# Richard-coder/uvio

Hardware: AMD Instinct MI355X
Metric: VIO frames/sec (track+propagate+update) at clones x feats (higher is better)
Workload: dtype f64

## Files before the change

include/uvio_hp.h:

```cpp
#ifndef UVIO_HP_H
#define UVIO_HP_H

#include <stddef.h>
#include <stdint.h>

#ifdef __cplusplus
extern "C" {
#endif

#define UVIO_HP_OK 0
#define UVIO_HP_E_ARG (-1)
#define UVIO_HP_E_STATE (-2)
#define UVIO_HP_E_DEVICE (-3)
#define UVIO_HP_E_NUMERIC (-4)
#define UVIO_HP_E_CONFIG (-5)
#define UVIO_HP_E_ORDER (-6)
#define UVIO_HP_E_CAPACITY (-7)
#define UVIO_HP_E_INTERNAL (-8)

#define UVIO_HP_MAX_CAMS 4
#define UVIO_HP_MAX_ANCHORS 16


typedef struct {
// ... 156 lines not shown
int uvio_hp_marginalize_slam(uvio_hp_t *h);
int uvio_hp_marginalize_old_clone(uvio_hp_t *h);
int uvio_hp_uwb_update_single(uvio_hp_t *h, double t, uint64_t anchor_id, double range, int *applied);

typedef int (*uvio_hp_allreduce_fn)(double *buf, size_t count, void *user);
int uvio_hp_shard_unique_id(uint8_t id[128]);
int uvio_hp_shard_init_rccl(uvio_hp_t *h, int rank, int world, const uint8_t id[128], int min_features);
int uvio_hp_shard_init_host(uvio_hp_t *h, int rank, int world, uvio_hp_allreduce_fn fn, void *user,
                            int min_features);
int uvio_hp_shard_partition(const int *rows, int n, int world, int *bounds);

int uvio_hp_debug_last_msckf(uvio_hp_t *h, uint64_t *ids, double *pG, int *status, double *chi2, int cap, int *n);
int uvio_hp_debug_frame_feats(uvio_hp_t *h, int *kind, uint64_t *ids, double *pG, int *status, double *chi2, int cap,
                              int *n);
int uvio_hp_ekf_update(double *P, int N, const int *H_index, int n, const double *H, int r,
                       const double *res, double sigma2, double *dx_out);
int uvio_hp_msckf_compressed_update(double *P, int N, const int *H_index, int n, const double *H, int m,
                                    const double *res, double sigma2, double *dx_out);
int uvio_hp_compress(const double *A, int m, int n, double *R_out);
int uvio_hp_undistort(int model, const double cam[8], int n, const float *uv, float *uvn, uint8_t *ambiguous);
int uvio_hp_debug_grid_order(const uint8_t *resp, const int *off, int ncell, int kmax, int depth, int *arrangement,
                             int *top);
int uvio_hp_debug_clahe(const uint8_t *img, int w, int h, int stride, uint8_t *out);
int uvio_hp_debug_grid_stats(uvio_hp_t *h, uint64_t *cells, uint64_t *introsort_cells);

#ifdef __cplusplus
}
#endif
#endif
```

uvio_amd/_native.py:

```python
import ctypes as C
import os

ROOT = os.path.dirname(os.path.dirname(os.path.abspath(__file__)))
LIB_PATH = os.environ.get("UVIO_HP_LIB", os.path.join(ROOT, "uvio_amd", "libuvio_hp.so"))

MAX_CAMS = 4
MAX_ANCHORS = 16

OK = 0
E_ARG, E_STATE, E_DEVICE, E_NUMERIC, E_CONFIG, E_ORDER, E_CAPACITY, E_INTERNAL = -1, -2, -3, -4, -5, -6, -7, -8
ERRNAMES = {0: "OK", -1: "E_ARG", -2: "E_STATE", -3: "E_DEVICE", -4: "E_NUMERIC", -5: "E_CONFIG", -6: "E_ORDER",
            -7: "E_CAPACITY", -8: "E_INTERNAL"}


class Camera(C.Structure):
    _fields_ = [("model", C.c_int), ("width", C.c_int), ("height", C.c_int), ("intrinsics", C.c_double * 8),
                ("q_ItoC", C.c_double * 4), ("p_IinC", C.c_double * 3)]


class Anchor(C.Structure):
    _fields_ = [("id", C.c_uint64), ("fix", C.c_int), ("p_AinG", C.c_double * 3), ("const_bias", C.c_double),
                ("dist_bias", C.c_double), ("cov_diag", C.c_double * 5)]


# ... 99 lines not shown
    ("get_tracks", _I, [C.c_void_p, _I, _P(C.c_uint64), _P(C.c_float), _I, _P(_I)]),
    ("get_pyramid", _I, [C.c_void_p, _I, _I, _P(_I), _P(_I), _P(C.c_uint8), _P(C.c_int16), C.c_size_t]),
    ("debug_last_msckf", _I, [C.c_void_p, _P(C.c_uint64), _P(_D), _P(_I), _P(_D), _I, _P(_I)]),
    ("debug_frame_feats", _I, [C.c_void_p, _P(_I), _P(C.c_uint64), _P(_D), _P(_I), _P(_D), _I, _P(_I)]),
    ("ekf_update", _I, [_P(_D), _I, _P(_I), _I, _P(_D), _I, _P(_D), _D, _P(_D)]),
    ("msckf_compressed_update", _I, [_P(_D), _I, _P(_I), _I, _P(_D), _I, _P(_D), _D, _P(_D)]),
    ("compress", _I, [_P(_D), _I, _I, _P(_D)]),
    ("undistort", _I, [_I, _P(_D), _I, _P(C.c_float), _P(C.c_float), _P(C.c_uint8)]),
    ("set_state", _I, [C.c_void_p, _P(_D), _P(_D), _I, _P(_D), _I, _I]),
    ("propagate_and_clone", _I, [C.c_void_p, _D]),
    ("msckf_update", _I, [C.c_void_p, _I, _P(C.c_uint64), _P(_I), _P(FeatMeas), _P(FeatResult)]),
    ("slam_update", _I, [C.c_void_p, _I, _P(C.c_uint64), _P(_I), _P(FeatMeas), _P(FeatResult)]),
    ("slam_delayed_init", _I, [C.c_void_p, _I, _P(C.c_uint64), _P(_I), _P(FeatMeas), _P(FeatResult)]),
    ("slam_change_anchors", _I, [C.c_void_p]),
    ("marginalize_slam", _I, [C.c_void_p]),
    ("marginalize_old_clone", _I, [C.c_void_p]),
    ("uwb_update_single", _I, [C.c_void_p, _D, C.c_uint64, _D, _P(_I)]),
    ("shard_unique_id", _I, [_P(C.c_uint8)]),
    ("shard_init_rccl", _I, [C.c_void_p, _I, _I, _P(C.c_uint8), _I]),
    ("shard_init_host", _I, [C.c_void_p, _I, _I, C.c_void_p, C.c_void_p, _I]),
    ("shard_partition", _I, [_P(_I), _I, _I, _P(_I)]),
    ("debug_grid_order", _I, [_P(C.c_uint8), _P(_I), _I, _I, _I, _P(_I), _P(_I)]),
    ("debug_clahe", _I, [_P(C.c_uint8), _I, _I, _I, _P(C.c_uint8)]),
    ("debug_grid_stats", _I, [C.c_void_p, _P(C.c_uint64), _P(C.c_uint64)]),
]

ALLREDUCE_FN = C.CFUNCTYPE(C.c_int, _P(_D), C.c_size_t, C.c_void_p)

EXPORTED = ["uvio_hp_" + s[0] for s in SIGNATURES]


MISSING = set()


def bind(lib, prefix, names=None):
    ab_old = os.environ.get("UVIO_HP_AB_OLD") == "1" and "UVIO_HP_LIB" in os.environ
    for name, res, args in SIGNATURES:
        if names is not None and name not in names:
            continue
        if ab_old and prefix == "uvio_hp_" and not hasattr(lib, prefix + name):
            MISSING.add(name)
            continue
        f = getattr(lib, prefix + name)
        f.restype = res
        f.argtypes = args
    if MISSING:
# ... 32 lines not shown
```

uvio_amd/csrc/capi.cpp:

```cpp
#include <cstring>
#include <string>

#include "engine.h"

using namespace uvhp;

struct uvio_hp {
  Engine *e = nullptr;
  std::string err;
  std::string fatal;
};

static std::string internal_error(const uvio_hp *h, const std::exception &ex) {
  std::string m = std::string("internal error: ") + ex.what();
  if (h && h->e && h->e->stage()[0]) m += std::string(" (in ") + h->e->stage() + ")";
  return m;
}

#define HP_GUARD(h, body)                                    \
  try {                                                      \
    if ((h) && (h)->e) HP_HIP(hipSetDevice((h)->e->device())); \
    body                                                     \
  } catch (const HpError &ex) {                              \
    if (h) (h)->err = ex.what();                             \
// ... 344 lines not shown
}

int uvio_hp_undistort(int model, const double cam[8], int n, const float *uv, float *uvn, uint8_t *ambiguous) {
  try {
    return Engine::undistort_standalone(model, cam, n, uv, uvn, ambiguous);
  } catch (const HpError &ex) {
    return ex.code;
  } catch (...) {
    return UVIO_HP_E_DEVICE;
  }
}

int uvio_hp_debug_grid_order(const uint8_t *resp, const int *off, int ncell, int kmax, int depth, int *arrangement,
                             int *top) {
  try {
    return Engine::grid_order_standalone(resp, off, ncell, kmax, depth, arrangement, top);
  } catch (const HpError &ex) {
    return ex.code;
  } catch (...) {
    return UVIO_HP_E_DEVICE;
  }
}

int uvio_hp_debug_clahe(const uint8_t *img, int w, int h, int stride, uint8_t *out) {
  try {
    return Engine::clahe_standalone(img, w, h, stride, out);
  } catch (const HpError &ex) {
    return ex.code;
  } catch (...) {
    return UVIO_HP_E_DEVICE;
  }
}

int uvio_hp_debug_grid_stats(uvio_hp_t *h, uint64_t *cells, uint64_t *introsort_cells) {
  if (!h) return UVIO_HP_E_ARG;
  unsigned long long c = 0;
  unsigned long long i = 0;
  HP_GUARD(h, if (h->e->tracker()) h->e->tracker()->grid_stats(&c, &i);)
  if (cells) *cells = c;
  if (introsort_cells) *introsort_cells = i;
  return 0;
}

}
```

uvio_amd/csrc/engine.h:

```cpp
#pragma once
#include <chrono>
#include <atomic>
#include <functional>
#include <map>
#include <memory>
#include <mutex>
#include <stdexcept>
#include <unordered_map>
#include <algorithm>
#include <cstdlib>
#include <vector>

#include "hp_common.h"
#include "hprof.h"
#include "kernels.h"
#include "pool.h"
#include "tracker.h"

namespace uvhp {

enum VKind { V_IMU = 0, V_VEC = 1, V_QUAT = 2, V_POSE = 3, V_LANDMARK = 4, V_ANCHOR = 5 };

struct Var {
  VKind kind;
// ... 335 lines not shown
  const Var &imu() const { return *imu_; }
  int cov_dim() const { return N_; }
  void get_cov(double *out, int ld);
  int state_vector(double *out, int cap, int *meta, int meta_cap, int *nvars, bool fej = false);
  uvio_hp_timing_t timing() const { return timing_; }
  std::vector<double> clone_times() const;

  void set_kernel_timing(int period) {
    ktime_period_ = period;
    kprof_.on = period > 0 && frames_ % period == 0;
  }
  void kernel_stats(bool flush, uvio_hp_kstat_t *out, int cap, int *n);

  void shard_init_rccl(int rank, int world, const uint8_t id[128], int min_features);
  void shard_init_host(int rank, int world, uvio_hp_allreduce_fn fn, void *user, int min_features);

  static int ekf_update_standalone(double *P, int N, const int *H_index, int n, const double *H, int r, const double *res,
                                   double sigma2, double *dx_out, bool compress = false);
  static int compress_standalone(const double *A, int m, int n, double *R_out);
  static int undistort_standalone(int model, const double cam[8], int n, const float *uv, float *uvn, uint8_t *amb);
  static int grid_order_standalone(const uint8_t *resp, const int *off, int ncell, int kmax, int depth,
                                   int *arrangement, int *top);
  static int clahe_standalone(const uint8_t *img, int w, int h, int stride, uint8_t *out);

 private:
  uvio_hp_options_t o_;
  int device_;
  DeviceBufs d_;
  double timestamp_ = -1;
  VarP imu_, calib_dt_, dw_, da_, tg_, qg_, qa_, p_IinU_;
  std::map<double, VarP> clones_;
  std::unordered_map<size_t, VarP> slam_;
  std::unordered_map<size_t, VarP> calib_pose_, calib_intr_;
  std::unordered_map<size_t, VarP> anchors_;
  CamParams cams_[UVIO_HP_MAX_CAMS];
  std::vector<VarP> vars_;
  int N_ = 0;
  long long p_epoch_ = 0;
  double early_prop_s_ = 0.0;
  std::mutex imu_mtx_;
  std::vector<ImuSample> imu_data_;
  bool have_last_prop_time_offset_ = false;
  double last_prop_time_offset_ = 0;
  std::unique_ptr<Tracker> tracker_;
  NodeSlabs db_nodes_;
  DbMap db_{SlabAlloc<std::pair<const size_t, FeatP>>(&db_nodes_)};
// ... 240 lines not shown
```

uvio_amd/csrc/engine_state.cpp:

```cpp
#include <sys/stat.h>

#include <algorithm>
#include <cstdio>
#include <cstring>

#include "engine.h"

namespace uvhp {

void Var::update(const double *dx) {
  if (kind == V_IMU || kind == V_POSE || kind == V_QUAT) {
    quat_boxplus(val, dx);
    for (int i = 3; i < size; i++) val[i + 1] += dx[i];
  } else {
    for (int i = 0; i < size; i++) val[i] += dx[i];
  }
}

void Var::xyz(bool getfej, double *o) const {
  const double *p = getfej ? fej : val;
  switch (rep) {
    case 0:
    case 2:
      o[0] = p[0]; o[1] = p[1]; o[2] = p[2];
// ... 950 lines not shown
  const size_t n = (size_t)w * h;
  ProbeScope ps;
  uint8_t *d_src = ps.alloc<uint8_t>(n), *d_img = ps.alloc<uint8_t>(n);
  int16_t *d_der = ps.alloc<int16_t>(2 * n);
  PyrJob job{};
  job.ncam = 1;
  job.method = 2;
  job.p[0].levels = 1;
  job.p[0].w[0] = w;
  job.p[0].h[0] = h;
  job.p[0].img[0] = d_img;
  job.p[0].der[0] = d_der;
  job.src[0] = d_src;
  job.stride[0] = w;
  job.clahe[0] = ps.alloc<uint8_t>(kClaheLutBytes);
  HP_HIP(hipMemcpy2DAsync(d_src, w, img, stride, w, h, hipMemcpyHostToDevice, ps.s));
  launch_pyramids(ps.s, job);
  HP_HIP(hipGetLastError());
  HP_HIP(hipMemcpyAsync(out, d_img, n, hipMemcpyDeviceToHost, ps.s));
  HP_HIP(hipStreamSynchronize(ps.s));
  return 0;
}

}
```

uvio_amd/csrc/kernels.h:

```cpp
#pragma once
#include <hip/hip_runtime.h>

#include <cstdint>

#include "hp_math.h"
#include "kprof.h"

namespace uvhp {

constexpr int kMaxMeasPerFeat = 64;
constexpr int kMaxVarsPerFeat = 48;
constexpr int kMaxCams = 4;

struct DClone {
  double R[9], p[3];
  double Rf[9], pf[3];
  int pid;
  int canon;
  int pad[2];
};

struct DCam {
  double R_ItoC[9], p_IinC[3];
  CamParams cam;
// ... 54 lines not shown
  const double *xv;
  int *gate_out;
};

void launch_cov_propagate(hipStream_t s, double *P, int ld, int N, int s0, int p, const int *iold, int q,
                          const double *Phi, const double *Q, double *T, const int *rows = nullptr);
void launch_clone(hipStream_t s, double *P, int ld, int N, int src0, int dt_id, const double *dnc_dev, int do_dt);
bool launch_prop_clone(hipStream_t s, double *P, int ld, int N, int s0, int p, const int *iold, int q,
                       const double *Phi, const double *Q, double *T, int src0, int dt_id, const double *dnc_dev,
                       int do_dt);
void launch_marginalize(hipStream_t s, const double *P, double *Pout, int ld, int N, int m0, int ms);
void launch_compact(hipStream_t s, const double *P, double *Pout, int ld, int Nn, const int *src);
void launch_marginalize_multi(hipStream_t s, const double *P, double *Pout, int ld, int Nn, const int *src);
void launch_check_diag(hipStream_t s, const double *P, int ld, int N, int *neg);

void launch_feature_linearize(hipStream_t s, const DBatchParams &bp, const DFeat *feats, const DMeas *meas,
                              const DVar *vars, const DClone *clones, const DCam *cams, const double *P,
                              const double *chi2_table, double *H_all, DFeatOut *out, int max_meas, int max_nf);
void launch_chi2_batch(hipStream_t s, const DBatchParams &bp, const DFeat *feats, const double *P, const int *hidx,
                       double *H_all, int m, double *T_all, const double *chi2_table, DFeatOut *out, int max_rows_f,
                       int *acc_count, double *pcan = nullptr,
                       double **sbuf = nullptr, size_t *sbuf_cap = nullptr);
size_t feature_lds_bytes(int max_meas, int max_nf);

void launch_gram(hipStream_t s, const double *A, int m, int ncol, int ldh, double *partials, int *nchunks_out);
int gram_num_chunks(int m);
void launch_shard_pack(hipStream_t s, const double *partials, int nch, int ncol, const DFeatOut *fout, int nf,
                       const int *acc, double *buf);
void launch_shard_unpack(hipStream_t s, const double *buf, int ncol, int *acc);
void launch_gram_reduce_chol(hipStream_t s, const double *partials, int nchunks, int ncol, double *R, int ldr);

constexpr int kMaxEkfRows = 255;
constexpr int kMaxDynLds = 152 * 1024;
constexpr int kUwbMaxRanges = 16;
struct DUwbState {
  double q[4], p[3];
  double pU[3];
  double anc[kUwbMaxRanges][5];
  double range[kUwbMaxRanges];
  int id_imu, id_cal;
  int id_anc[kUwbMaxRanges];
  int nr;
};
void launch_uwb_row(hipStream_t s, DUwbState *st, int j, const double *prev, double *h, double *region);
void launch_uwb_M(hipStream_t s, const double *P, int ldp, int N, const double *h, const int *hidx, int n, double *M);
void launch_uwb_update(hipStream_t s, double *P, int ldp, int N, const double *M, const double *h, const int *hidx,
// ... 175 lines not shown
```

uvio_amd/csrc/kernels_feat.hip:

```cpp
#include <stdexcept>
#include <string>

#include "kernels.h"

namespace uvhp {

__device__ __forceinline__ double wave_sum(double v) {
#pragma unroll
  for (int o = 32; o > 0; o >>= 1) v += __shfl_xor(v, o, 64);
  return v;
}
__device__ __forceinline__ void wave_sync() {
  __builtin_amdgcn_fence(__ATOMIC_RELEASE, "wavefront");
  __builtin_amdgcn_wave_barrier();
  __builtin_amdgcn_fence(__ATOMIC_ACQUIRE, "wavefront");
}
template <int NV>
__device__ __forceinline__ void ordered_sum(double *red, const double *v, int lane, int m, double *out) {
  wave_sync();
#pragma unroll
  for (int k = 0; k < NV; k++) red[lane * NV + k] = v[k];
  wave_sync();
  if (lane < NV) {
    double s = 0.0;
// ... 92 lines not shown
#pragma unroll
      for (int i = k + 1; i < 3; i++) s += A[3 * i + j] * A[3 * i + j];
      cn[j] = s;
    }
  }
  double y[3] = {0, 0, 0};
#pragma unroll
  for (int i = 2; i >= 0; i--) {
    if (i < rank) {
      double v = b[i];
#pragma unroll
      for (int k = i + 1; k < 3; k++)
        if (k < rank) v -= A[3 * i + k] * y[k];
      y[i] = v / A[3 * i + i];
    }
  }
#pragma unroll
  for (int i = 0; i < 3; i++)
#pragma unroll
    for (int j = 0; j < 3; j++)
      if (perm[i] == j) x[j] = y[i];
}

__device__ void singular_values3(const double *A, double *sv) {
  double a[3][3];
  for (int i = 0; i < 3; i++)
    for (int j = 0; j < 3; j++) a[i][j] = A[i] * A[j] + A[3 + i] * A[3 + j] + A[6 + i] * A[6 + j];
  for (int sweep = 0; sweep < 60; sweep++) {
    double off = a[0][1] * a[0][1] + a[0][2] * a[0][2] + a[1][2] * a[1][2];
    if (off < 1e-300 || off <= 1e-36 * (a[0][0] * a[0][0] + a[1][1] * a[1][1] + a[2][2] * a[2][2])) break;
    for (int p = 0; p < 2; p++)
      for (int q = p + 1; q < 3; q++) {
        if (a[p][q] == 0) continue;
        double theta = (a[q][q] - a[p][p]) / (2 * a[p][q]);
        double t = (theta >= 0 ? 1.0 : -1.0) / (fabs(theta) + sqrt(theta * theta + 1));
        double c = 1 / sqrt(t * t + 1), s = t * c;
        for (int k = 0; k < 3; k++) {
          double akp = a[k][p], akq = a[k][q];
          a[k][p] = c * akp - s * akq;
          a[k][q] = s * akp + c * akq;
        }
        for (int k = 0; k < 3; k++) {
          double apk = a[p][k], aqk = a[q][k];
          a[p][k] = c * apk - s * aqk;
          a[q][k] = s * apk + c * aqk;
        }
      }
// ... 80 lines not shown
        w1[q] = a1[q];
        w2[q] = a2[q];
        w3[q] = a3[q];
      } else {
        w1[q] = __shfl(a1[q / TPC], base + q % TPC, 64);
        w2[q] = __shfl(a2[q / TPC], base + q % TPC, 64);
        w3[q] = __shfl(a3[q / TPC], base + q % TPC, 64);
      }
    }
    const double s1 = (w1[0] + w1[1]) + (w1[2] + w1[3]);
    const double s2 = (w2[0] + w2[1]) + (w2[2] + w2[3]);
    const double s3 = (w3[0] + w3[1]) + (w3[2] + w3[3]);
    const double u1 = b1 * s1;
    const double u2 = b2 * (s2 - g21 * u1);
    const double u3 = b3 * (s3 - g31 * u1 - g32 * u2);
#pragma unroll 4
    for (int k = part; k < rows; k += TPC) {
      double *p = Hl + (size_t)k * ldl + j;
      *p -= V[k * 3] * u1 + V[k * 3 + 1] * u2 + V[k * 3 + 2] * u3;
    }
  }
}

struct FeatShared {
  double p_FinA[3], p_FinG[3], p_FinA_fej[3], p_FinG_fej[3];
  int status;
  int nrows_out;
  double beta[3];
  double chi2;
};

__host__ __device__ inline size_t feat_lds_doubles(int max_meas, int max_nf) {
  int rows = 2 * max_meas;
  size_t n = 0;
  n += (size_t)rows * (max_nf + 1);
  n += (size_t)rows * 3;
  n += (size_t)rows * 3;
  n += (size_t)max_nf;
  n += 64;
  return n;
}
size_t feature_lds_bytes(int max_meas, int max_nf) { return feat_lds_doubles(max_meas, max_nf) * sizeof(double); }

__global__ void __launch_bounds__(256) k_feature(DBatchParams bp, const DFeat *__restrict__ feats,
                                                 const DMeas *__restrict__ meas, const DVar *__restrict__ vars,
                                                 const DClone *__restrict__ clones, const DCam *__restrict__ cams,
                                                 const double *__restrict__ P, const double *__restrict__ chi2_table,
                                                 double *__restrict__ H_all, DFeatOut *__restrict__ out, int max_meas,
                                                 int max_nf) {
  extern __shared__ double lds[];
  __shared__ FeatShared sh;
  long long *tsp = bp.dbg_ts ? bp.dbg_ts + (size_t)blockIdx.x * 16 : nullptr;
#define FEAT_TS(k) \
  if (tsp && threadIdx.x == 0) tsp[k] = clock64();
  __shared__ int canon2loc[512];
  __shared__ double red[9 * 64 + 16];
  const int f = blockIdx.x;
  const DFeat F = feats[f];
  const int m = F.nmeas, rows = 2 * m, nf = F.nf, ldl = nf + 1;
  const int tid = threadIdx.x, lane = tid & 63, wave = tid >> 6;
  const DMeas *Ms = meas + F.meas_off;

  double *Hl = lds;
  double *Hf = Hl + (size_t)2 * max_meas * (max_nf + 1);
  double *V = Hf + 2 * max_meas * 3;
  int *loc2pid = (int *)(V + 2 * max_meas * 3);

  FEAT_TS(0)
  for (int j = tid; j <= bp.n_canon; j += 256) canon2loc[j] = -1;
  for (int e = tid; e < rows * ldl; e += 256) Hl[e] = 0.0;
  __syncthreads();
  for (int e = tid; e < F.nvar * 8; e += 256) {
    const DVar dv = vars[F.var_off + (e >> 3)];
    const int k = e & 7;
    if (k < dv.size) {
      loc2pid[dv.loc + k] = dv.pid + k;
      if (dv.canon >= 0) canon2loc[dv.canon + k] = dv.loc + k;
    }
  }
  if (tid == 0) {
    sh.status = 0;
    double pin[3], pinf[3];
    for (int k = 0; k < 3; k++) pin[k] = F.p_in[k], pinf[k] = F.p_in_fej[k];
    if (F.mode == 3 && bp.tri_in) {
      const DFeatOut &t = bp.tri_in[f];
      for (int k = 0; k < 3; k++) pin[k] = t.p_FinA[k], pinf[k] = t.p_FinG[k];
      if (t.status == 1 || t.status == 2) sh.status = 1;
    }
    if (F.mode == 1 && bp.xv && F.lm_pid >= 0) {
      const double *v = bp.xv + F.lm_pid;
      if (F.rep == 4) {
        pin[0] = (1 / v[2]) * v[0];
        pin[1] = (1 / v[2]) * v[1];
        pin[2] = 1 / v[2];
        for (int k = 0; k < 3; k++) pinf[k] = pin[k];
      } else {
        for (int k = 0; k < 3; k++) pin[k] = v[k];
      }
    }
    for (int k = 0; k < 3; k++) {
// ... 364 lines not shown
        if (bp.calib_ext)
          for (int j = 0; j < 6; j++)
            row[F.lc_anchor_ext + j] +=
                dz_dpfg[3 * i] * Hcal[j] + dz_dpfg[3 * i + 1] * Hcal[6 + j] + dz_dpfg[3 * i + 2] * Hcal[12 + j];
      }
      if (bp.calib_ext && mm.lc_ext >= 0) {
        double pc[3] = {p_FinCi[0] - ck.p_IinC[0], p_FinCi[1] - ck.p_IinC[1], p_FinCi[2] - ck.p_IinC[2]}, Sc[9];
        skew(pc, Sc);
        for (int j = 0; j < 3; j++) {
          row[mm.lc_ext + j] += dz_dpfc[3 * i] * Sc[j] + dz_dpfc[3 * i + 1] * Sc[3 + j] + dz_dpfc[3 * i + 2] * Sc[6 + j];
          row[mm.lc_ext + 3 + j] += dz_dpfc[3 * i + j];
        }
      }
      if (bp.calib_intr && mm.lc_intr >= 0)
        for (int j = 0; j < 8; j++) row[mm.lc_intr + j] = dzeta[8 * i + j];
      row[nf] = (i == 0) ? res0 : res1;
      if (F.mode == 1)
        for (int j = 0; j < ncolf; j++) row[F.lm_loc + j] = hf[j];
    }
  }
  __syncthreads();

  FEAT_TS(3)
  int r0 = 0;
  if (status0 == 0 && F.mode != 1) {
    if (wave == 0) {
      for (int c = 0; c < 3; c++) {
        double ss = 0.0;
        for (int i = c + lane; i < rows; i += 64) {
          double x = Hf[i * 3 + c];
          ss += x * x;
        }
        ss = wave_sum(ss);
        const double x0 = Hf[c * 3 + c];
        const double alpha = (x0 > 0) ? -sqrt(ss) : sqrt(ss);
        for (int i = lane; i < rows; i += 64) {
          V[i * 3 + c] = (i < c) ? 0.0 : (i == c) ? (x0 - alpha) : Hf[i * 3 + c];
          if (i >= c) Hf[i * 3 + c] = (i == c) ? alpha : 0.0;
        }
        const double vn = ss - x0 * x0 + (x0 - alpha) * (x0 - alpha);
        const double b = (vn > 0) ? 2.0 / vn : 0.0;
        if (lane == 0) sh.beta[c] = b;
        wave_sync();
        for (int j = c + 1; j < 3; j++) {
          double d = 0.0;
          for (int i = c + lane; i < rows; i += 64) d += V[i * 3 + c] * Hf[i * 3 + j];
          d = b * wave_sum(d);
          for (int i = c + lane; i < rows; i += 64) Hf[i * 3 + j] -= d * V[i * 3 + c];
        }
        wave_sync();
      }
      double g0 = 0.0, g1 = 0.0, g2 = 0.0;
      for (int i = lane; i < rows; i += 64) {
        const double a = V[i * 3], bq = V[i * 3 + 1], cq = V[i * 3 + 2];
        g0 += bq * a;
        g1 += cq * a;
        g2 += cq * bq;
      }
      g0 = wave_sum(g0);
      g1 = wave_sum(g1);
      g2 = wave_sum(g2);
      if (lane == 0) red[0] = g0, red[1] = g1, red[2] = g2;
      if (F.mode == 3) FEAT_TS(8)
    }
    __syncthreads();
    if (F.mode == 3) FEAT_TS(9)
    const double b1 = sh.beta[0], b2 = sh.beta[1], b3 = sh.beta[2];
    const double g21 = red[0], g31 = red[1], g32 = red[2];
    if (ldl <= 64)
      ns_apply<4>(Hl, V, rows, ldl, tid, b1, b2, b3, g21, g31, g32);
    else if (ldl <= 128)
      ns_apply<2>(Hl, V, rows, ldl, tid, b1, b2, b3, g21, g31, g32);
    else
      ns_apply<1>(Hl, V, rows, ldl, tid, b1, b2, b3, g21, g31, g32);
    if (F.mode == 3) FEAT_TS(10)
    __syncthreads();
    r0 = 3;
  }
  const int R = rows - r0;

  FEAT_TS(4)
  FEAT_TS(5)
  const int status = sh.status;
  FEAT_TS(6)
  const int out_r0 = (F.mode == 0) ? 3 : 0;
  const int nrows_out = max(rows - out_r0, 0);
  {
    const int nc = bp.n_canon + 1;
    int lcs[8];
#pragma unroll
    for (int q = 0; q < 8; q++) {
      const int j = lane + 64 * q;
      lcs[q] = (status != 0 || j >= nc) ? -1 : (j == bp.n_canon) ? nf : canon2loc[j];
    }
    for (int i = wave; i < nrows_out; i += 4) {
      const double *src = Hl + (size_t)(out_r0 + i) * ldl;
      double *dst = H_all + (size_t)(F.row_off + i) * bp.ldh;
#pragma unroll
      for (int q = 0; q < 8; q++) {
        const int j = lane + 64 * q;
        if (j < nc) dst[j] = (lcs[q] >= 0) ? src[lcs[q]] : 0.0;
      }
    }
  }
  if (tid == 0) {
    DFeatOut o;
    for (int k = 0; k < 3; k++) {
      o.p_FinA[k] = sh.p_FinA[k];
      o.p_FinG[k] = sh.p_FinG[k];
    }
    o.chi2 = -1.0;
    for (int k = 0; k < 9; k++) o.HfR[k] = (F.mode >= 2 && status0 == 0) ? Hf[(k / 3) * 3 + (k % 3)] : 0.0;
    o.status = status;
    o.rows = status == 0 ? nrows_out : 0;
    out[f] = o;
    if (bp.gate_out) *bp.gate_out = (status == 0) ? 1 : 0;
  }
  FEAT_TS(7)
#undef FEAT_TS
}

void launch_feature_linearize(hipStream_t s, const DBatchParams &bp, const DFeat *feats, const DMeas *meas,
                              const DVar *vars, const DClone *clones, const DCam *cams, const double *P,
                              const double *chi2_table, double *H_all, DFeatOut *out, int max_meas, int max_nf) {
  if (bp.nfeat <= 0) return;
  if (bp.n_canon >= 512 || max_meas > 64)
    throw std::runtime_error("k_feature: n_canon " + std::to_string(bp.n_canon) + " / measurements per feature " +
                             std::to_string(max_meas) + " beyond the kernel's limits (511 / 64)");
  size_t bytes = feature_lds_bytes(max_meas, max_nf);
  static int granted = -1;
  if (granted < 0) granted = set_dyn_lds((const void *)k_feature, 156 * 1024);
  if (bytes > 64 * 1024 && (int)bytes > granted)
    throw std::runtime_error("k_feature needs " + std::to_string(bytes) + " B of LDS, granted " + std::to_string(granted));
  hipLaunchKernelGGL(k_feature, dim3(bp.nfeat), dim3(256), bytes, s, bp, feats, meas, vars, clones, cams, P,
                     chi2_table, H_all, out, max_meas, max_nf);
}

__device__ __forceinline__ unsigned retri_hash(unsigned long long k, int cap) {
  k ^= k >> 33;
  k *= 0xff51afd7ed558ccdull;
  k ^= k >> 33;
  return (unsigned)(k & (unsigned long long)(cap - 1));
}
__device__ int retri_find(const unsigned long long *keys, int cap, unsigned long long id) {
  unsigned h = retri_hash(id, cap);
  for (int p = 0; p < cap; p++, h = (h + 1) & (cap - 1)) {
    const unsigned long long k = keys[h];
    if (k == id) return (int)h;
    if (k == kRetriEmpty) return -1;
  }
  return -1;
}
__device__ int retri_insert(unsigned long long *keys, int cap, unsigned long long id) {
  unsigned h = retri_hash(id, cap);
  for (int p = 0; p < cap; p++, h = (h + 1) & (cap - 1)) {
    const unsigned long long prev = atomicCAS(&keys[h], kRetriEmpty, id);
    if (prev == kRetriEmpty || prev == id) return (int)h;
  }
// ... 143 lines not shown
```

uvio_amd/manager.py:

```python
import ctypes as C

import numpy as np

from . import _native as N


def load_options(yaml_path=None, **overrides):
    lib = N.load()
    opts = N.Options()
    N.check(lib.uvio_hp_options_default(C.byref(opts)), what="options_default")
    if yaml_path is not None:
        N.check(lib.uvio_hp_options_load(yaml_path.encode(), C.byref(opts)), what="options_load(%s)" % yaml_path)
    apply_overrides(opts, overrides)
    return opts


def _mask_ptrs(masks, ncam):
    mk = [None if m is None else np.ascontiguousarray(m, dtype=np.uint8) for m in masks]
    ptrs = [C.POINTER(C.c_uint8)() if m is None else m.ctypes.data_as(C.POINTER(C.c_uint8)) for m in mk]
    return mk, (C.POINTER(C.c_uint8) * ncam)(*ptrs)


def apply_overrides(opts, overrides):
    for k, v in overrides.items():
# ... 393 lines not shown
    N.check(lib.uvio_hp_compress(_dp(A), m, nc - 1, _dp(R)), what="uvio_hp_compress")
    return R


def grid_order(cells, kmax=0, depth=-1):
    lib = N.load()
    off = np.zeros(len(cells) + 1, dtype=np.int32)
    for i, c in enumerate(cells):
        off[i + 1] = off[i] + len(c)
    resp = np.zeros(max(int(off[-1]), 1), dtype=np.uint8)
    for i, c in enumerate(cells):
        resp[off[i]:off[i + 1]] = np.asarray(c, dtype=np.int64)
    arr = np.zeros(max(int(off[-1]), 1), dtype=np.int32)
    top = np.full(max(len(cells) * kmax, 1), -1, dtype=np.int32)
    ip = C.POINTER(C.c_int)
    rc = lib.uvio_hp_debug_grid_order(resp.ctypes.data_as(C.POINTER(C.c_uint8)), off.ctypes.data_as(ip), len(cells),
                                      kmax, depth, arr.ctypes.data_as(ip), top.ctypes.data_as(ip))
    N.check(rc, what="uvio_hp_debug_grid_order")
    arrs = [arr[off[i]:off[i + 1]].copy() for i in range(len(cells))]
    tops = [top[i * kmax:i * kmax + min(kmax, len(c))].copy() for i, c in enumerate(cells)] if kmax > 0 else None
    return arrs, tops


def clahe(img):
    lib = N.load()
    img = np.asarray(img)
    if img.ndim != 2 or img.dtype != np.uint8:
        raise ValueError("clahe: a 2-D uint8 image")
    if img.strides[1] != 1 or img.strides[0] < img.shape[1]:
        img = np.ascontiguousarray(img)
    h, w = img.shape
    out = np.zeros((h, w), dtype=np.uint8)
    bp = C.POINTER(C.c_uint8)
    rc = lib.uvio_hp_debug_clahe(img.ctypes.data_as(bp), w, h, img.strides[0], out.ctypes.data_as(bp))
    N.check(rc, what="uvio_hp_debug_clahe")
    return out


def undistort(cam, uv, return_ambiguous=False):
    lib = N.load()
    uv = np.ascontiguousarray(uv, dtype=np.float32).reshape(-1, 2)
    out = np.zeros_like(uv)
    amb = np.zeros(uv.shape[0], dtype=np.uint8)
    intr = np.array(cam.intrinsics[:], dtype=np.float64)
    fp = C.POINTER(C.c_float)
    rc = lib.uvio_hp_undistort(int(cam.model), _dp(intr), uv.shape[0], uv.ctypes.data_as(fp), out.ctypes.data_as(fp),
# ... 4 lines not shown
```

Baseline: 1067.

## Apply nullspace projection from registers and scatter directly to H_all

Adds a register-resident path for the three-reflector Householder nullspace projection in k_feature. Each wave holds a quarter of the rows for up to four 64-column blocks and exchanges partial reflector sums through LDS, then writes projected rows straight into canonical H_all columns instead of writing back to LDS and running a separate scatter pass. k_feature is templated on row and column capacity and dispatched from a table, with an env var to force the old LDS path. A standalone probe API is added for testing, and the register footprint per template may affect occupancy.

```diff
diff --git a/include/uvio_hp.h b/include/uvio_hp.h
--- a/include/uvio_hp.h
+++ b/include/uvio_hp.h
@@ -202,6 +202,9 @@
 int uvio_hp_debug_grid_order(const uint8_t *resp, const int *off, int ncell, int kmax, int depth, int *arrangement,
                              int *top);
 int uvio_hp_debug_clahe(const uint8_t *img, int w, int h, int stride, uint8_t *out);
+int uvio_hp_debug_ns_project(const double *A, int rows, int ldl, const double *V, const double beta[3],
+                             const double g[3], const int *loc2canon, int n_canon, int out_r0, int variant,
+                             int status, double *out);
 int uvio_hp_debug_grid_stats(uvio_hp_t *h, uint64_t *cells, uint64_t *introsort_cells);
 
 #ifdef __cplusplus
diff --git a/uvio_amd/_native.py b/uvio_amd/_native.py
--- a/uvio_amd/_native.py
+++ b/uvio_amd/_native.py
@@ -145,6 +145,7 @@
     ("shard_partition", _I, [_P(_I), _I, _I, _P(_I)]),
     ("debug_grid_order", _I, [_P(C.c_uint8), _P(_I), _I, _I, _I, _P(_I), _P(_I)]),
     ("debug_clahe", _I, [_P(C.c_uint8), _I, _I, _I, _P(C.c_uint8)]),
+    ("debug_ns_project", _I, [_P(_D), _I, _I, _P(_D), _P(_D), _P(_D), _P(_I), _I, _I, _I, _I, _P(_D)]),
     ("debug_grid_stats", _I, [C.c_void_p, _P(C.c_uint64), _P(C.c_uint64)]),
 ]
 
diff --git a/uvio_amd/csrc/capi.cpp b/uvio_amd/csrc/capi.cpp
--- a/uvio_amd/csrc/capi.cpp
+++ b/uvio_amd/csrc/capi.cpp
@@ -390,6 +390,18 @@
   }
 }
 
+int uvio_hp_debug_ns_project(const double *A, int rows, int ldl, const double *V, const double beta[3],
+                             const double g[3], const int *loc2canon, int n_canon, int out_r0, int variant,
+                             int status, double *out) {
+  try {
+    return Engine::ns_project_standalone(A, rows, ldl, V, beta, g, loc2canon, n_canon, out_r0, variant, status, out);
+  } catch (const HpError &ex) {
+    return ex.code;
+  } catch (...) {
+    return UVIO_HP_E_DEVICE;
+  }
+}
+
 int uvio_hp_debug_clahe(const uint8_t *img, int w, int h, int stride, uint8_t *out) {
   try {
     return Engine::clahe_standalone(img, w, h, stride, out);
diff --git a/uvio_amd/csrc/engine.h b/uvio_amd/csrc/engine.h
--- a/uvio_amd/csrc/engine.h
+++ b/uvio_amd/csrc/engine.h
@@ -381,6 +381,9 @@
   static int grid_order_standalone(const uint8_t *resp, const int *off, int ncell, int kmax, int depth,
                                    int *arrangement, int *top);
   static int clahe_standalone(const uint8_t *img, int w, int h, int stride, uint8_t *out);
+  static int ns_project_standalone(const double *A, int rows, int ldl, const double *V, const double beta[3],
+                                   const double g[3], const int *loc2canon, int n_canon, int out_r0, int variant,
+                                   int status, double *out);
 
  private:
   uvio_hp_options_t o_;
diff --git a/uvio_amd/csrc/engine_state.cpp b/uvio_amd/csrc/engine_state.cpp
--- a/uvio_amd/csrc/engine_state.cpp
+++ b/uvio_amd/csrc/engine_state.cpp
@@ -996,4 +996,38 @@
   return 0;
 }
 
-}
+int Engine::ns_project_standalone(const double *A, int rows, int ldl, const double *V, const double beta[3],
+                                  const double g[3], const int *loc2canon, int n_canon, int out_r0, int variant,
+                                  int status, double *out) {
+  if (!A || !V || !beta || !g || !loc2canon || !out || variant < 0 || variant > 4 || out_r0 < 0 || n_canon < 0)
+    return UVIO_HP_E_ARG;
+  if (rows < 2 || rows > 128 || (rows & 1) || ldl < 2 || ldl > 512 || n_canon >= 512) return UVIO_HP_E_CAPACITY;
+  if (variant >= 2 && (ldl > 64 * variant || rows < 12)) return UVIO_HP_E_ARG;
+  std::vector<char> seen(n_canon, 0);
+  for (int j = 0; j + 1 < ldl; j++) {
+    const int c = loc2canon[j];
+    if (c >= n_canon || (c >= 0 && seen[c]++)) return UVIO_HP_E_ARG;
+  }
+  if (loc2canon[ldl - 1] != n_canon) return UVIO_HP_E_ARG;
+  int ndev = 0;
+  if (hipGetDeviceCount(&ndev) != hipSuccess || ndev < 1) return UVIO_HP_E_DEVICE;
+  const size_t nA = (size_t)rows * ldl, nout = (size_t)std::max(rows - out_r0, 0) * (n_canon + 1);
+  if (nout == 0) return 0;
+  ProbeScope ps;
+  double *d_A = ps.alloc<double>(nA), *d_work = ps.alloc<double>(nA), *d_V = ps.alloc<double>((size_t)rows * 3);
+  double *d_bg = ps.alloc<double>(6), *d_out = ps.alloc<double>(nout);
+  int *d_map = ps.alloc<int>(ldl);
+  const double bg[6] = {beta[0], beta[1], beta[2], g[0], g[1], g[2]};
+  HP_HIP(hipMemcpyAsync(d_A, A, sizeof(double) * nA, hipMemcpyHostToDevice, ps.s));
+  HP_HIP(hipMemcpyAsync(d_V, V, sizeof(double) * rows * 3, hipMemcpyHostToDevice, ps.s));
+  HP_HIP(hipMemcpyAsync(d_bg, bg, sizeof(bg), hipMemcpyHostToDevice, ps.s));
+  HP_HIP(hipMemcpyAsync(d_map, loc2canon, sizeof(int) * ldl, hipMemcpyHostToDevice, ps.s));
+  HP_HIP(hipMemsetAsync(d_out, 0xff, sizeof(double) * nout, ps.s));
+  launch_ns_project_probe(ps.s, d_A, d_work, d_V, d_bg, d_map, rows, ldl, n_canon, out_r0, variant, status, d_out);
+  HP_HIP(hipGetLastError());
+  HP_HIP(hipMemcpyAsync(out, d_out, sizeof(double) * nout, hipMemcpyDeviceToHost, ps.s));
+  HP_HIP(hipStreamSynchronize(ps.s));
+  return 0;
+}
+
+}
diff --git a/uvio_amd/csrc/kernels.h b/uvio_amd/csrc/kernels.h
--- a/uvio_amd/csrc/kernels.h
+++ b/uvio_amd/csrc/kernels.h
@@ -100,6 +100,9 @@
                        int *acc_count, double *pcan = nullptr,
                        double **sbuf = nullptr, size_t *sbuf_cap = nullptr);
 size_t feature_lds_bytes(int max_meas, int max_nf);
+void launch_ns_project_probe(hipStream_t s, const double *d_A, double *d_work, const double *d_V, const double *d_bg,
+                             const int *d_loc2canon, int rows, int ldl, int n_canon, int out_r0, int variant,
+                             int status, double *d_out);
 
 void launch_gram(hipStream_t s, const double *A, int m, int ncol, int ldh, double *partials, int *nchunks_out);
 int gram_num_chunks(int m);
diff --git a/uvio_amd/csrc/kernels_feat.hip b/uvio_amd/csrc/kernels_feat.hip
--- a/uvio_amd/csrc/kernels_feat.hip
+++ b/uvio_amd/csrc/kernels_feat.hip
@@ -138,7 +138,7 @@
       if (perm[i] == j) x[j] = y[i];
 }
 
-__device__ void singular_values3(const double *A, double *sv) {
+__device__ __forceinline__ void singular_values3(const double *A, double *sv) {
   double a[3][3];
   for (int i = 0; i < 3; i++)
     for (int j = 0; j < 3; j++) a[i][j] = A[i] * A[j] + A[3 + i] * A[3 + j] + A[6 + i] * A[6 + j];
@@ -265,6 +265,237 @@
   }
 }
 
+
+__host__ __device__ inline int ns_reg_cb(int rows, int ldl, int cbmax) {
+  return (rows < 12 || ldl <= 64 || ldl > 64 * cbmax) ? 0 : (ldl + 63) / 64;
+}
+
+__device__ __forceinline__ void ns_zero_cols(const int *canon2loc, int n_canon, double *dst0, int ldh, int nrows_out,
+                                             int w, int nw, int lane) {
+  bool z[8];
+#pragma unroll
+  for (int q = 0; q < 8; q++) {
+    const int j = lane + 64 * q;
+    z[q] = j < n_canon && canon2loc[j] < 0;
+  }
+  for (int i = w; i < nrows_out; i += nw) {
+    double *dst = dst0 + (size_t)i * ldh;
+#pragma unroll
+    for (int q = 0; q < 8; q++)
+      if (z[q]) dst[lane + 64 * q] = 0.0;
+  }
+}
+
+template <int RQ, int CB>
+__device__ __forceinline__ void ns_reg_load(double (&a)[RQ][CB], const double *Hl, int nq, int ldl, int part, int col0) {
+  auto row = [&](int k) {
+    const double *src = Hl + (size_t)(4 * k + part) * ldl;
+#pragma unroll
+    for (int c = 0; c < CB; c++) a[k][c] = src[min(col0 + 64 * c, ldl - 1)];
+  };
+#pragma unroll
+  for (int k0 = 0; k0 < RQ; k0 += 4) {
+    if (k0 + 4 <= nq) {
+#pragma unroll
+      for (int k = k0; k < k0 + 4; k++) row(k);
+    } else {
+#pragma unroll
+      for (int k = k0; k < k0 + 4; k++) {
+        if (k < nq) {
+          row(k);
+        } else {
+#pragma unroll
+          for (int c = 0; c < CB; c++) a[k][c] = 0.0;
+        }
+      }
+    }
+  }
+}
+
+template <int RQ, int CB>
+__device__ __forceinline__ void ns_reg_apply(double (&a)[RQ][CB], double *Hl, const double *V, int rows, int ldl,
+                                             int part, int col0, double b1, double b2, double b3, double g21,
+                                             double g31, double g32, const int (&cn)[CB], double *dst0, int ldh,
+                                             int out_r0, long long *ts) {
+  const int rows4 = rows & ~3, nq = rows4 >> 2;
+  double a1[CB], a2[CB], a3[CB];
+#pragma unroll
+  for (int c = 0; c < CB; c++) a1[c] = a2[c] = a3[c] = 0.0;
+  auto sum_row = [&](int k) {
+    const double *v = V + (4 * k + part) * 3;
+    const double v1 = v[0], v2 = v[1], v3 = v[2];
+#pragma unroll
+    for (int c = 0; c < CB; c++) {
+      a1[c] += v1 * a[k][c];
+      a2[c] += v2 * a[k][c];
+      a3[c] += v3 * a[k][c];
+    }
+  };
+#pragma unroll
+  for (int k0 = 0; k0 < RQ; k0 += 4) {
+    if (k0 + 4 <= nq) {
+#pragma unroll
+      for (int k = k0; k < k0 + 4; k++) sum_row(k);
+    } else {
+#pragma unroll
+      for (int k = k0; k < k0 + 4; k++)
+        if (k < nq) sum_row(k);
+    }
+  }
+  if (part == 0)
+    for (int r = rows4; r < rows; r++) {
+      const double v1 = V[r * 3], v2 = V[r * 3 + 1], v3 = V[r * 3 + 2];
+#pragma unroll
+      for (int c = 0; c < CB; c++) {
+        const int j = col0 + 64 * c;
+        const double x = (j < ldl) ? Hl[(size_t)r * ldl + j] : 0.0;
+        a1[c] += v1 * x;
+        a2[c] += v2 * x;
+        a3[c] += v3 * x;
+      }
+    }
+  double *xch = Hl;
+#pragma unroll
+  for (int c = 0; c < CB; c++) {
+    const int j = col0 + 64 * c;
+    if (j < ldl) {
+      xch[(size_t)(3 * part) * ldl + j] = a1[c];
+      xch[(size_t)(3 * part + 1) * ldl + j] = a2[c];
+      xch[(size_t)(3 * part + 2) * ldl + j] = a3[c];
+    }
+  }
+  __syncthreads();
+  if (ts && threadIdx.x == 0) ts[11] = clock64();
+  double u1[CB], u2[CB], u3[CB];
+#pragma unroll
+  for (int c = 0; c < CB; c++) {
+    const double *w = xch + min(col0 + 64 * c, ldl - 1);
+    const double s1 = (w[0] + w[(size_t)3 * ldl]) + (w[(size_t)6 * ldl] + w[(size_t)9 * ldl]);
+    const double s2 = (w[(size_t)ldl] + w[(size_t)4 * ldl]) + (w[(size_t)7 * ldl] + w[(size_t)10 * ldl]);
+    const double s3 = (w[(size_t)2 * ldl] + w[(size_t)5 * ldl]) + (w[(size_t)8 * ldl] + w[(size_t)11 * ldl]);
+    u1[c] = b1 * s1;
+    u2[c] = b2 * (s2 - g21 * u1[c]);
+    u3[c] = b3 * (s3 - g31 * u1[c] - g32 * u2[c]);
+  }
+  asm volatile("" ::: "memory");
+  auto out_row = [&](int k) {
+    const int r = 4 * k + part;
+    const double v1 = V[r * 3], v2 = V[r * 3 + 1], v3 = V[r * 3 + 2];
+    double *dst = dst0 + ((ptrdiff_t)r - out_r0) * ldh;
+#pragma unroll
+    for (int c = 0; c < CB; c++) {
+      const double x = a[k][c] - (v1 * u1[c] + v2 * u2[c] + v3 * u3[c]);
+      if (r >= out_r0 && cn[c] >= 0) dst[cn[c]] = x;
+    }
+  };
+#pragma unroll
+  for (int k0 = 0; k0 < RQ; k0 += 4) {
+    if (k0 + 4 <= nq) {
+#pragma unroll
+      for (int k = k0; k < k0 + 4; k++) out_row(k);
+    } else {
+#pragma unroll
+      for (int k = k0; k < k0 + 4; k++)
+        if (k < nq) out_row(k);
+    }
+  }
+  const int rt = rows4 + part - 2;
+  if (part >= 2 && rt < rows && rt >= out_r0) {
+    const double v1 = V[rt * 3], v2 = V[rt * 3 + 1], v3 = V[rt * 3 + 2];
+    double *dst = dst0 + (size_t)(rt - out_r0) * ldh;
+#pragma unroll
+    for (int c = 0; c < CB; c++)
+      if (cn[c] >= 0) dst[cn[c]] = Hl[(size_t)rt * ldl + col0 + 64 * c] - (v1 * u1[c] + v2 * u2[c] + v3 * u3[c]);
+  }
+}
+
+__device__ __forceinline__ void ns_reflectors(double *Hf, double *V, int rows, int lane, double *beta, double *g) {
+  for (int c = 0; c < 3; c++) {
+    double ss = 0.0;
+    for (int i = c + lane; i < rows; i += 64) {
+      double x = Hf[i * 3 + c];
+      ss += x * x;
+    }
+    ss = wave_sum(ss);
+    const double x0 = Hf[c * 3 + c];
+    const double alpha = (x0 > 0) ? -sqrt(ss) : sqrt(ss);
+    for (int i = lane; i < rows; i += 64) {
+      V[i * 3 + c] = (i < c) ? 0.0 : (i == c) ? (x0 - alpha) : Hf[i * 3 + c];
+      if (i >= c) Hf[i * 3 + c] = (i == c) ? alpha : 0.0;
+    }
+    const double vn = ss - x0 * x0 + (x0 - alpha) * (x0 - alpha);
+    const double b = (vn > 0) ? 2.0 / vn : 0.0;
+    if (lane == 0) beta[c] = b;
+    wave_sync();
+    for (int j = c + 1; j < 3; j++) {
+      double d = 0.0;
+      for (int i = c + lane; i < rows; i += 64) d += V[i * 3 + c] * Hf[i * 3 + j];
+      d = b * wave_sum(d);
+      for (int i = c + lane; i < rows; i += 64) Hf[i * 3 + j] -= d * V[i * 3 + c];
+    }
+    wave_sync();
+  }
+  double g0 = 0.0, g1 = 0.0, g2 = 0.0;
+  for (int i = lane; i < rows; i += 64) {
+    const double a = V[i * 3], bq = V[i * 3 + 1], cq = V[i * 3 + 2];
+    g0 += bq * a;
+    g1 += cq * a;
+    g2 += cq * bq;
+  }
+  g0 = wave_sum(g0);
+  g1 = wave_sum(g1);
+  g2 = wave_sum(g2);
+  if (lane == 0) g[0] = g0, g[1] = g1, g[2] = g2;
+}
+
+template <int RQ, int CB>
+__device__ __forceinline__ void ns_project_reg(double *Hl, double *Hf, double *V, double *beta, double *g,
+                                               int rows, int ldl, int tid, const int *canon2loc,
+                                               const int *loc2canon, int n_canon, double *dst0, int ldh, int out_r0,
+                                               long long *ts) {
+  const int lane = tid & 63, wave = tid >> 6, part = wave, col0 = lane, nf = ldl - 1;
+  const int nq = (rows & ~3) >> 2;
+  double a[RQ][CB];
+  int cn[CB];
+#pragma unroll
+  for (int c = 0; c < CB; c++) {
+    const int j = col0 + 64 * c;
+    cn[c] = (j < nf) ? loc2canon[j] : (j == nf) ? n_canon : -1;
+  }
+  if (wave == 0 && Hf) {
+    ns_reflectors(Hf, V, rows, lane, beta, g);
+    if (ts && lane == 0) ts[8] = clock64();
+  }
+  ns_reg_load<RQ, CB>(a, Hl, nq, ldl, part, col0);
+  if (wave != 0) ns_zero_cols(canon2loc, n_canon, dst0, ldh, max(rows - out_r0, 0), wave - 1, 3, lane);
+  __syncthreads();
+  if (ts && tid == 0) ts[9] = clock64();
+  ns_reg_apply<RQ, CB>(a, Hl, V, rows, ldl, part, col0, beta[0], beta[1], beta[2], g[0], g[1], g[2], cn, dst0, ldh,
+                       out_r0, ts);
+  if (ts && tid == 0) ts[10] = clock64();
+}
+
+__device__ __forceinline__ void ns_write_rows_lds(const double *Hl, int ldl, const int *canon2loc, int n_canon,
+                                                  int status, double *dst0, int ldh, int out_r0, int nrows_out,
+                                                  int lane, int wave) {
+  const int nc = n_canon + 1, nf = ldl - 1;
+  int lcs[8];
+#pragma unroll
+  for (int q = 0; q < 8; q++) {
+    const int j = lane + 64 * q;
+    lcs[q] = (status != 0 || j >= nc) ? -1 : (j == n_canon) ? nf : canon2loc[j];
+  }
+  for (int i = wave; i < nrows_out; i += 4) {
+    const double *src = Hl + (size_t)(out_r0 + i) * ldl;
+    double *dst = dst0 + (size_t)i * ldh;
+#pragma unroll
+    for (int q = 0; q < 8; q++) {
+      const int j = lane + 64 * q;
+      if (j < nc) dst[j] = (lcs[q] >= 0) ? src[lcs[q]] : 0.0;
+    }
+  }
+}
+
 struct FeatShared {
   double p_FinA[3], p_FinG[3], p_FinA_fej[3], p_FinG_fej[3];
   int status;
@@ -285,12 +516,13 @@
 }
 size_t feature_lds_bytes(int max_meas, int max_nf) { return feat_lds_doubles(max_meas, max_nf) * sizeof(double); }
 
+template <int RQ, int CBMAX>
 __global__ void __launch_bounds__(256) k_feature(DBatchParams bp, const DFeat *__restrict__ feats,
                                                  const DMeas *__restrict__ meas, const DVar *__restrict__ vars,
                                                  const DClone *__restrict__ clones, const DCam *__restrict__ cams,
                                                  const double *__restrict__ P, const double *__restrict__ chi2_table,
                                                  double *__restrict__ H_all, DFeatOut *__restrict__ out, int max_meas,
-                                                 int max_nf) {
+                                                 int max_nf, int ns_lds) {
   extern __shared__ double lds[];
   __shared__ FeatShared sh;
   long long *tsp = bp.dbg_ts ? bp.dbg_ts + (size_t)blockIdx.x * 16 : nullptr;
@@ -308,9 +540,11 @@
   double *Hf = Hl + (size_t)2 * max_meas * (max_nf + 1);
   double *V = Hf + 2 * max_meas * 3;
   int *loc2pid = (int *)(V + 2 * max_meas * 3);
+  int *loc2canon = loc2pid + max_nf;
 
   FEAT_TS(0)
   for (int j = tid; j <= bp.n_canon; j += 256) canon2loc[j] = -1;
+  for (int j = tid; j < nf; j += 256) loc2canon[j] = -1;
   for (int e = tid; e < rows * ldl; e += 256) Hl[e] = 0.0;
   __syncthreads();
   for (int e = tid; e < F.nvar * 8; e += 256) {
@@ -318,7 +552,7 @@
     const int k = e & 7;
     if (k < dv.size) {
       loc2pid[dv.loc + k] = dv.pid + k;
-      if (dv.canon >= 0) canon2loc[dv.canon + k] = dv.loc + k;
+      if (dv.canon >= 0) canon2loc[dv.canon + k] = dv.loc + k, loc2canon[dv.loc + k] = dv.canon + k;
     }
   }
   if (tid == 0) {
@@ -729,45 +963,23 @@
   __syncthreads();
 
   FEAT_TS(3)
-  int r0 = 0;
-  if (status0 == 0 && F.mode != 1) {
+  const int out_r0 = (F.mode == 0) ? 3 : 0;
+  const int nrows_out = max(rows - out_r0, 0);
+  double *const dst0 = H_all + (size_t)F.row_off * bp.ldh;
+  const int cb = (status0 == 0 && F.mode != 1 && !ns_lds) ? ns_reg_cb(rows, ldl, CBMAX) : 0;
+  long long *const ts3 = (F.mode == 3) ? tsp : nullptr;
+  if (CBMAX >= 2 && cb == 2) {
+    ns_project_reg<RQ, 2>(Hl, Hf, V, sh.beta, red, rows, ldl, tid, canon2loc, loc2canon, bp.n_canon, dst0, bp.ldh,
+                          out_r0, ts3);
+  } else if (CBMAX >= 3 && cb == 3) {
+    ns_project_reg<RQ, 3>(Hl, Hf, V, sh.beta, red, rows, ldl, tid, canon2loc, loc2canon, bp.n_canon, dst0, bp.ldh,
+                          out_r0, ts3);
+  } else if (CBMAX >= 4 && cb == 4) {
+    ns_project_reg<RQ, 4>(Hl, Hf, V, sh.beta, red, rows, ldl, tid, canon2loc, loc2canon, bp.n_canon, dst0, bp.ldh,
+                          out_r0, ts3);
+  } else if (status0 == 0 && F.mode != 1) {
     if (wave == 0) {
-      for (int c = 0; c < 3; c++) {
-        double ss = 0.0;
-        for (int i = c + lane; i < rows; i += 64) {
-          double x = Hf[i * 3 + c];
-          ss += x * x;
-        }
-        ss = wave_sum(ss);
-        const double x0 = Hf[c * 3 + c];
-        const double alpha = (x0 > 0) ? -sqrt(ss) : sqrt(ss);
-        for (int i = lane; i < rows; i += 64) {
-          V[i * 3 + c] = (i < c) ? 0.0 : (i == c) ? (x0 - alpha) : Hf[i * 3 + c];
-          if (i >= c) Hf[i * 3 + c] = (i == c) ? alpha : 0.0;
-        }
-        const double vn = ss - x0 * x0 + (x0 - alpha) * (x0 - alpha);
-        const double b = (vn > 0) ? 2.0 / vn : 0.0;
-        if (lane == 0) sh.beta[c] = b;
-        wave_sync();
-        for (int j = c + 1; j < 3; j++) {
-          double d = 0.0;
-          for (int i = c + lane; i < rows; i += 64) d += V[i * 3 + c] * Hf[i * 3 + j];
-          d = b * wave_sum(d);
-          for (int i = c + lane; i < rows; i += 64) Hf[i * 3 + j] -= d * V[i * 3 + c];
-        }
-        wave_sync();
-      }
-      double g0 = 0.0, g1 = 0.0, g2 = 0.0;
-      for (int i = lane; i < rows; i += 64) {
-        const double a = V[i * 3], bq = V[i * 3 + 1], cq = V[i * 3 + 2];
-        g0 += bq * a;
-        g1 += cq * a;
-        g2 += cq * bq;
-      }
-      g0 = wave_sum(g0);
-      g1 = wave_sum(g1);
-      g2 = wave_sum(g2);
-      if (lane == 0) red[0] = g0, red[1] = g1, red[2] = g2;
+      ns_reflectors(Hf, V, rows, lane, sh.beta, red);
       if (F.mode == 3) FEAT_TS(8)
     }
     __syncthreads();
@@ -782,34 +994,13 @@
       ns_apply<1>(Hl, V, rows, ldl, tid, b1, b2, b3, g21, g31, g32);
     if (F.mode == 3) FEAT_TS(10)
     __syncthreads();
-    r0 = 3;
-  }
-  const int R = rows - r0;
+  }
 
   FEAT_TS(4)
   FEAT_TS(5)
   const int status = sh.status;
   FEAT_TS(6)
-  const int out_r0 = (F.mode == 0) ? 3 : 0;
-  const int nrows_out = max(rows - out_r0, 0);
-  {
-    const int nc = bp.n_canon + 1;
-    int lcs[8];
-#pragma unroll
-    for (int q = 0; q < 8; q++) {
-      const int j = lane + 64 * q;
-      lcs[q] = (status != 0 || j >= nc) ? -1 : (j == bp.n_canon) ? nf : canon2loc[j];
-    }
-    for (int i = wave; i < nrows_out; i += 4) {
-      const double *src = Hl + (size_t)(out_r0 + i) * ldl;
-      double *dst = H_all + (size_t)(F.row_off + i) * bp.ldh;
-#pragma unroll
-      for (int q = 0; q < 8; q++) {
-        const int j = lane + 64 * q;
-        if (j < nc) dst[j] = (lcs[q] >= 0) ? src[lcs[q]] : 0.0;
-      }
-    }
-  }
+  if (cb == 0) ns_write_rows_lds(Hl, ldl, canon2loc, bp.n_canon, status, dst0, bp.ldh, out_r0, nrows_out, lane, wave);
   if (tid == 0) {
     DFeatOut o;
     for (int k = 0; k < 3; k++) {
@@ -835,12 +1026,84 @@
     throw std::runtime_error("k_feature: n_canon " + std::to_string(bp.n_canon) + " / measurements per feature " +
                              std::to_string(max_meas) + " beyond the kernel's limits (511 / 64)");
   size_t bytes = feature_lds_bytes(max_meas, max_nf);
-  static int granted = -1;
-  if (granted < 0) granted = set_dyn_lds((const void *)k_feature, 156 * 1024);
-  if (bytes > 64 * 1024 && (int)bytes > granted)
-    throw std::runtime_error("k_feature needs " + std::to_string(bytes) + " B of LDS, granted " + std::to_string(granted));
-  hipLaunchKernelGGL(k_feature, dim3(bp.nfeat), dim3(256), bytes, s, bp, feats, meas, vars, clones, cams, P,
-                     chi2_table, H_all, out, max_meas, max_nf);
+  using Fn = decltype(&k_feature<8, 0>);
+  static const Fn fns[3][4] = {{k_feature<8, 0>, k_feature<8, 0>, k_feature<8, 0>, k_feature<8, 0>},
+                               {k_feature<8, 0>, k_feature<16, 2>, k_feature<24, 2>, k_feature<32, 2>},
+                               {k_feature<8, 0>, k_feature<16, 4>, k_feature<24, 4>, k_feature<32, 4>}};
+  static int granted[3][4] = {{-1, -1, -1, -1}, {-1, -1, -1, -1}, {-1, -1, -1, -1}};
+  static const int ns_lds = std::getenv("UVIO_HP_NS_LDS") != nullptr;
+  const int wc = (max_nf + 1 <= 64) ? 0 : (max_nf + 1 <= 128) ? 1 : 2;
+  const int rc = wc == 0 ? 0 : std::max(max_meas - 1, 0) / 16;
+  if (granted[wc][rc] < 0) granted[wc][rc] = set_dyn_lds((const void *)fns[wc][rc], 156 * 1024);
+  if (bytes > 64 * 1024 && (int)bytes > granted[wc][rc])
+    throw std::runtime_error("k_feature needs " + std::to_string(bytes) + " B of LDS, granted " +
+                             std::to_string(granted[wc][rc]));
+  hipLaunchKernelGGL(fns[wc][rc], dim3(bp.nfeat), dim3(256), bytes, s, bp, feats, meas, vars, clones, cams, P,
+                     chi2_table, H_all, out, max_meas, max_nf, ns_lds);
+}
+
+template <int RQ>
+__global__ void __launch_bounds__(256) k_ns_project_probe(const double *__restrict__ A, double *work,
+                                                          const double *__restrict__ Vin, const double *__restrict__ bg,
+                                                          const int *__restrict__ loc2canon_in, int rows, int ldl,
+                                                          int n_canon, int out_r0, int cb, int status,
+                                                          double *__restrict__ outp) {
+  extern __shared__ double lds[];
+  __shared__ int canon2loc[512], loc2canon[512];
+  __shared__ double beta[3], g[3];
+  const int tid = threadIdx.x, lane = tid & 63, wave = tid >> 6, nf = ldl - 1;
+  double *V = lds;
+  double *Hl = work ? work : lds + (size_t)rows * 3;
+  for (int j = tid; j <= n_canon; j += 256) canon2loc[j] = -1;
+  for (int j = tid; j < nf; j += 256) loc2canon[j] = loc2canon_in[j];
+  for (int e = tid; e < rows * ldl; e += 256) Hl[e] = A[e];
+  for (int e = tid; e < rows * 3; e += 256) V[e] = Vin[e];
+  if (tid < 3) beta[tid] = bg[tid], g[tid] = bg[3 + tid];
+  __syncthreads();
+  for (int j = tid; j < nf; j += 256)
+    if (loc2canon[j] >= 0) canon2loc[loc2canon[j]] = j;
+  __syncthreads();
+  const int nrows_out = max(rows - out_r0, 0), ldh = n_canon + 1;
+  if (status != 0) cb = 0;
+  if (cb == 2) {
+    ns_project_reg<RQ, 2>(Hl, nullptr, V, beta, g, rows, ldl, tid, canon2loc, loc2canon, n_canon, outp, ldh, out_r0,
+                          nullptr);
+  } else if (cb == 3) {
+    ns_project_reg<RQ, 3>(Hl, nullptr, V, beta, g, rows, ldl, tid, canon2loc, loc2canon, n_canon, outp, ldh, out_r0,
+                          nullptr);
+  } else if (cb == 4) {
+    ns_project_reg<RQ, 4>(Hl, nullptr, V, beta, g, rows, ldl, tid, canon2loc, loc2canon, n_canon, outp, ldh, out_r0,
+                          nullptr);
+  } else if (status == 0) {
+    if (ldl <= 64)
+      ns_apply<4>(Hl, V, rows, ldl, tid, beta[0], beta[1], beta[2], g[0], g[1], g[2]);
+    else if (ldl <= 128)
+      ns_apply<2>(Hl, V, rows, ldl, tid, beta[0], beta[1], beta[2], g[0], g[1], g[2]);
+    else
+      ns_apply<1>(Hl, V, rows, ldl, tid, beta[0], beta[1], beta[2], g[0], g[1], g[2]);
+    __syncthreads();
+  }
+  if (cb == 0) ns_write_rows_lds(Hl, ldl, canon2loc, n_canon, status, outp, ldh, out_r0, nrows_out, lane, wave);
+}
+
+void launch_ns_project_probe(hipStream_t s, const double *d_A, double *d_work, const double *d_V, const double *d_bg,
+                             const int *d_loc2canon, int rows, int ldl, int n_canon, int out_r0, int variant,
+                             int status, double *d_out) {
+  if (rows < 2 || rows > 128 || (rows & 1) || ldl < 2 || ldl > 512 || n_canon < 0 || n_canon >= 512 || variant < 0 || variant > 4 ||
+      (variant >= 2 && (ldl > 64 * variant || rows < 12)))
+    throw std::runtime_error("k_ns_project_probe: shape or variant out of range");
+  using Fn = decltype(&k_ns_project_probe<8>);
+  static const Fn fns[4] = {k_ns_project_probe<8>, k_ns_project_probe<16>, k_ns_project_probe<24>,
+                            k_ns_project_probe<32>};
+  const int rc = (rows / 2 - 1) / 16;
+  const int cb = variant == 0 ? 0 : variant == 1 ? ns_reg_cb(rows, ldl, 4) : variant;
+  size_t bytes = sizeof(double) * ((size_t)rows * 3 + (size_t)rows * ldl);
+  const bool in_lds = bytes <= 150 * 1024;
+  if (!in_lds) bytes = sizeof(double) * (size_t)rows * 3;
+  if (bytes > 64 * 1024 && set_dyn_lds((const void *)fns[rc], (int)bytes) < (int)bytes)
+    throw std::runtime_error("k_ns_project_probe: LDS not granted");
+  hipLaunchKernelGGL(fns[rc], dim3(1), dim3(256), bytes, s, d_A, in_lds ? nullptr : d_work, d_V, d_bg, d_loc2canon,
+                     rows, ldl, n_canon, out_r0, cb, status, d_out);
 }
 
 __device__ __forceinline__ unsigned retri_hash(unsigned long long k, int cap) {
diff --git a/uvio_amd/manager.py b/uvio_amd/manager.py
--- a/uvio_amd/manager.py
+++ b/uvio_amd/manager.py
@@ -439,6 +439,23 @@
     return arrs, tops
 
 
+def ns_project(A, V, beta, g, loc2canon, n_canon, out_r0, variant, status=0):
+    lib = N.load()
+    A = np.ascontiguousarray(A, dtype=np.float64)
+    V = np.ascontiguousarray(V, dtype=np.float64)
+    beta = np.ascontiguousarray(beta, dtype=np.float64)
+    g = np.ascontiguousarray(g, dtype=np.float64)
+    l2c = np.ascontiguousarray(loc2canon, dtype=np.int32)
+    rows, ldl = A.shape
+    if V.shape != (rows, 3) or beta.shape != (3,) or g.shape != (3,) or l2c.shape != (ldl,):
+        raise ValueError("ns_project: V rows x 3, beta[3], g[3], loc2canon[ldl]")
+    out = np.full((max(rows - out_r0, 0), n_canon + 1), np.nan)
+    rc = lib.uvio_hp_debug_ns_project(_dp(A), rows, ldl, _dp(V), _dp(beta), _dp(g), l2c.ctypes.data_as(C.POINTER(C.c_int)),
+                                      int(n_canon), int(out_r0), int(variant), int(status), _dp(out))
+    N.check(rc, what="uvio_hp_debug_ns_project")
+    return out
+
+
 def clahe(img):
     lib = N.load()
     img = np.asarray(img)
```

Measured after the change: 1021. 4.4% lower.
